# HKUDS/LLMRec

Measured on NVIDIA H100. Metric: train_interactions_per_sec, higher is better.
Workload: dtype f32

## Files before the change

llmrec_b200/csrc/dispatch.cu:

```cuda
#include <vector>
#include "common.cuh"

namespace llmrec {
int proj_fwd_simt(const float*, int64_t, const float*, const float*, float*, int64_t, int64_t, int, int, const int*, cudaStream_t);
int proj_fwd_simt(const uint16_t*, int64_t, const float*, const float*, float*, int64_t, int64_t, int, int, const int*, cudaStream_t);
int proj_wgrad_simt(const float*, int64_t, const float*, int64_t, float*, float*, int64_t, int, int, int, const int*, int64_t, cudaStream_t);
int proj_wgrad_simt(const uint16_t*, int64_t, const float*, int64_t, float*, float*, int64_t, int, int, int, const int*, int64_t, cudaStream_t);
int score_topk_simt(const float*, int64_t, const float*, int64_t, const int*, int, int, int, const int*, const int*, int, int*, float*, float*, int64_t, cudaStream_t);
bool proj_tc_supported(int d, int64_t ldx, const void* X, int k, bool wgrad, bool bf16);
int proj_fwd_tc_group(const llmrec_proj_fwd_problem*, const int32_t* const*, int, int, int, bool, cudaStream_t);
int proj_wgrad_tc_group(const llmrec_proj_wgrad_problem*, const int32_t* const*, const int64_t*, int, int, int, bool, float*, int64_t, cudaStream_t);
int64_t proj_wgrad_tc_scratch(const llmrec_proj_wgrad_problem*, int, int, bool);
bool score_tc_supported(int d, int K, long long ldu, long long ldi, const void* U, const void* I);
long long score_tc_scratch(int n_batch, int n_items, int d, int K);
int score_topk_tc(const float*, long long, const float*, long long, const int*, int, int, int, const int*, const int*, int, int*, float*, float*, long long, cudaStream_t);
}
using namespace llmrec;

static bool fwd_tc_ok(const llmrec_proj_fwd_problem* pr, int n, int d, int mode, bool bf16) {
  if (mode == 2 || n > 8) return false;
  for (int p = 0; p < n; ++p)
    if (!proj_tc_supported(d, pr[p].ldx, pr[p].X, pr[p].k, false, bf16) || pr[p].ldy % 4 != 0 || !aligned16(pr[p].Y) || !aligned16(pr[p].W) ||
        (pr[p].bias && !aligned16(pr[p].bias)) || ((mode == 0 || bf16) && !pr[p].wsplit))
      return false;
  return true;
}
static bool wg_tc_ok(const llmrec_proj_wgrad_problem* pr, int n, int d, int mode, bool bf16) {
  if (mode == 2 || n > 8) return false;
  for (int p = 0; p < n; ++p)
    if (!proj_tc_supported(d, pr[p].ldx, pr[p].X, pr[p].k, true, bf16) || pr[p].lddy % 4 != 0 || !aligned16(pr[p].dY)) return false;
  return true;
}

struct RowMaps { std::vector<const int32_t*> rows; std::vector<int64_t> n_dy; };
static int32_t flags(const llmrec_proj_fwd_problem& p) { return p._reserved; }
static int32_t flags(const llmrec_proj_fwd_problem_bf16& p) { return p._reserved; }
static int32_t flags(const llmrec_proj_wgrad_problem& p) { return p.accumulate; }
static int32_t flags(const llmrec_proj_wgrad_problem_bf16& p) { return p.accumulate; }
template <class Prob>
static int row_maps(const Prob* pr, int32_t n_prob, bool wgrad, RowMaps& M) {
  bool any = false;
  for (int p = 0; p < n_prob; ++p) any = any || (flags(pr[p]) & LLMREC_PROJ_ROW_MAP);
  if (!any) return 0;
  const llmrec_proj_row_map* rec = reinterpret_cast<const llmrec_proj_row_map*>(pr + n_prob);
  M.rows.assign(n_prob, nullptr);
  M.n_dy.assign(n_prob, 0);
  for (int p = 0; p < n_prob; ++p) {
    M.n_dy[p] = pr[p].n;
    if (!(flags(pr[p]) & LLMREC_PROJ_ROW_MAP)) continue;
    LLMREC_CHECK_ARG(rec[p].rows || pr[p].n <= 0, "proj: problem %d is flagged LLMREC_PROJ_ROW_MAP but its map is NULL", p);
    LLMREC_CHECK_ARG(!wgrad || rec[p].n_dy >= 0, "proj_wgrad: problem %d has a negative dY row count", p);
    M.rows[p] = rec[p].rows; M.n_dy[p] = rec[p].n_dy;
  }
  return 0;
}

static int proj_fwd_group(const llmrec_proj_fwd_problem* pr, const int32_t* const* rows, int32_t n_prob, int32_t d, int32_t mode, bool bf16,
                          llmrec_stream_t stream) {
  LLMREC_REQUIRE_DEVICE();
  LLMREC_CHECK_ARG(n_prob >= 1 && d >= 1, "proj_fwd_group: bad sizes");
  cudaStream_t st = as_stream(stream);
  for (int p0 = 0; p0 < n_prob; p0 += 8) {
    int np = n_prob - p0 < 8 ? n_prob - p0 : 8;
    if (fwd_tc_ok(pr + p0, np, d, mode, bf16)) {
      int rc = proj_fwd_tc_group(pr + p0, rows ? rows + p0 : nullptr, np, d, mode, bf16, st);
      if (rc) return rc;
    } else {
      for (int p = p0; p < p0 + np; ++p) {
        if (pr[p].n <= 0) continue;
        const int32_t* map = rows ? rows[p] : nullptr;
        int rc = bf16 ? proj_fwd_simt(reinterpret_cast<const uint16_t*>(pr[p].X), pr[p].ldx, pr[p].W, pr[p].bias, pr[p].Y, pr[p].ldy, pr[p].n, pr[p].k, d, map, st)
                      : proj_fwd_simt(pr[p].X, pr[p].ldx, pr[p].W, pr[p].bias, pr[p].Y, pr[p].ldy, pr[p].n, pr[p].k, d, map, st);
        if (rc) return rc;
      }
    }
  }
  return 0;
}
static std::vector<llmrec_proj_fwd_problem> as_f32_layout(const llmrec_proj_fwd_problem_bf16* pr, int32_t n_prob) {
  std::vector<llmrec_proj_fwd_problem> q(n_prob > 0 ? n_prob : 0);
  for (int p = 0; p < n_prob; ++p)
    q[p] = {reinterpret_cast<const float*>(pr[p].X), pr[p].W, pr[p].bias, pr[p].Y, pr[p].wsplit, pr[p].ldx, pr[p].ldy, pr[p].n, pr[p].k, 0};
  return q;
}
extern "C" int llmrec_proj_fwd_group_f32(const llmrec_proj_fwd_problem* pr, int32_t n_prob, int32_t d, int32_t mode, llmrec_stream_t stream) {
  LLMREC_CHECK_ARG(pr && n_prob >= 1, "proj_fwd_group: bad sizes");
  RowMaps M;
  if (int rc = row_maps(pr, n_prob, false, M)) return rc;
  return proj_fwd_group(pr, M.rows.empty() ? nullptr : M.rows.data(), n_prob, d, mode, false, stream);
}
extern "C" int llmrec_proj_fwd_group_bf16(const llmrec_proj_fwd_problem_bf16* pr, int32_t n_prob, int32_t d, int32_t mode, llmrec_stream_t stream) {
  LLMREC_CHECK_ARG(pr && n_prob >= 1, "proj_fwd_group: bad sizes");
  RowMaps M;
  if (int rc = row_maps(pr, n_prob, false, M)) return rc;
  return proj_fwd_group(as_f32_layout(pr, n_prob).data(), M.rows.empty() ? nullptr : M.rows.data(), n_prob, d, mode, true, stream);
}
extern "C" int llmrec_proj_fwd_f32(const float* X, int64_t ldx, const float* W, const float* bias, float* Y, int64_t ldy,
                                   int64_t n, int32_t k, int32_t d, int32_t mode, float* wsplit, llmrec_stream_t stream) {
  llmrec_proj_fwd_problem p{X, W, bias, Y, wsplit, ldx, ldy, n, k, 0};
  if (n <= 0) return 0;
  return llmrec_proj_fwd_group_f32(&p, 1, d, mode, stream);
}

static int64_t proj_wgrad_scratch(const llmrec_proj_wgrad_problem* pr, int32_t n_prob, int32_t d, int32_t mode, bool bf16) {
  int64_t need = 0;
  for (int p0 = 0; p0 < n_prob; p0 += 8) {
    int np = n_prob - p0 < 8 ? n_prob - p0 : 8;
    if (wg_tc_ok(pr + p0, np, d, mode, bf16)) { int64_t s = proj_wgrad_tc_scratch(pr + p0, np, d, bf16); need = s > need ? s : need; }
  }
  return need;
}
static int proj_wgrad_group(const llmrec_proj_wgrad_problem* pr, const int32_t* const* rows, const int64_t* n_dy, int32_t n_prob, int32_t d,
                            int32_t mode, bool bf16, float* scratch, int64_t scratch_elems, llmrec_stream_t stream) {
  LLMREC_REQUIRE_DEVICE();
  LLMREC_CHECK_ARG(n_prob >= 1 && d >= 1, "proj_wgrad_group: bad sizes");
  cudaStream_t st = as_stream(stream);
  for (int p0 = 0; p0 < n_prob; p0 += 8) {
    int np = n_prob - p0 < 8 ? n_prob - p0 : 8;
    if (wg_tc_ok(pr + p0, np, d, mode, bf16)) {
      int rc = proj_wgrad_tc_group(pr + p0, rows ? rows + p0 : nullptr, rows ? n_dy + p0 : nullptr, np, d, mode, bf16, scratch, scratch_elems, st);
      if (rc) return rc;
    } else {
      for (int p = p0; p < p0 + np; ++p) {
        const int acc = pr[p].accumulate & LLMREC_WGRAD_ACCUMULATE;
        const int32_t* map = rows ? rows[p] : nullptr;
        const int64_t ndy = n_dy ? n_dy[p] : pr[p].n;
        int rc = bf16 ? proj_wgrad_simt(reinterpret_cast<const uint16_t*>(pr[p].X), pr[p].ldx, pr[p].dY, pr[p].lddy, pr[p].dW, pr[p].db, pr[p].n, pr[p].k, d, acc, map, ndy, st)
                      : proj_wgrad_simt(pr[p].X, pr[p].ldx, pr[p].dY, pr[p].lddy, pr[p].dW, pr[p].db, pr[p].n, pr[p].k, d, acc, map, ndy, st);
        if (rc) return rc;
      }
    }
  }
  return 0;
}
static std::vector<llmrec_proj_wgrad_problem> as_f32_layout(const llmrec_proj_wgrad_problem_bf16* pr, int32_t n_prob) {
  std::vector<llmrec_proj_wgrad_problem> q(n_prob > 0 ? n_prob : 0);
  for (int p = 0; p < n_prob; ++p)
    q[p] = {reinterpret_cast<const float*>(pr[p].X), pr[p].dY, pr[p].dW, pr[p].db, pr[p].ldx, pr[p].lddy, pr[p].n, pr[p].k, pr[p].accumulate};
  return q;
}
extern "C" int64_t llmrec_proj_wgrad_group_scratch(const llmrec_proj_wgrad_problem* pr, int32_t n_prob, int32_t d, int32_t mode) {
  return proj_wgrad_scratch(pr, n_prob, d, mode, false);
}
extern "C" int64_t llmrec_proj_wgrad_group_bf16_scratch(const llmrec_proj_wgrad_problem_bf16* pr, int32_t n_prob, int32_t d, int32_t mode) {
  return proj_wgrad_scratch(as_f32_layout(pr, n_prob).data(), n_prob, d, mode, true);
}
extern "C" int llmrec_proj_wgrad_group_f32(const llmrec_proj_wgrad_problem* pr, int32_t n_prob, int32_t d, int32_t mode,
                                           float* scratch, int64_t scratch_elems, llmrec_stream_t stream) {
  LLMREC_CHECK_ARG(pr && n_prob >= 1, "proj_wgrad_group: bad sizes");
  RowMaps M;
  if (int rc = row_maps(pr, n_prob, true, M)) return rc;
  const bool mapped = !M.rows.empty();
  return proj_wgrad_group(pr, mapped ? M.rows.data() : nullptr, mapped ? M.n_dy.data() : nullptr, n_prob, d, mode, false, scratch, scratch_elems, stream);
}
extern "C" int llmrec_proj_wgrad_group_bf16(const llmrec_proj_wgrad_problem_bf16* pr, int32_t n_prob, int32_t d, int32_t mode,
                                            float* scratch, int64_t scratch_elems, llmrec_stream_t stream) {
  LLMREC_CHECK_ARG(pr && n_prob >= 1, "proj_wgrad_group: bad sizes");
  RowMaps M;
  if (int rc = row_maps(pr, n_prob, true, M)) return rc;
  const bool mapped = !M.rows.empty();
  return proj_wgrad_group(as_f32_layout(pr, n_prob).data(), mapped ? M.rows.data() : nullptr, mapped ? M.n_dy.data() : nullptr, n_prob, d, mode,
                          true, scratch, scratch_elems, stream);
}
extern "C" int64_t llmrec_proj_wgrad_scratch(int64_t n, int32_t k, int32_t d, int32_t mode) {
  llmrec_proj_wgrad_problem p{nullptr, nullptr, nullptr, nullptr, 4, 4, n, k, 0};
  if (mode == 2 || d % 32 != 0 || d > 256 || k % 4 != 0) return 0;
  return proj_wgrad_tc_scratch(&p, 1, d, false);
}
extern "C" int llmrec_proj_wgrad_f32(const float* X, int64_t ldx, const float* dY, int64_t lddy, float* dW, float* db,
                                     int64_t n, int32_t k, int32_t d, int32_t accumulate, int32_t mode,
                                     float* scratch, int64_t scratch_elems, llmrec_stream_t stream) {
  llmrec_proj_wgrad_problem p{X, dY, dW, db, ldx, lddy, n, k, accumulate};
  return llmrec_proj_wgrad_group_f32(&p, 1, d, mode, scratch, scratch_elems, stream);
}

extern "C" int64_t llmrec_score_topk_scratch(int32_t n_batch, int32_t n_items, int32_t d, int32_t K, int32_t mode) {
  if (mode != 2 && (d == 32 || d == 64 || d == 96 || d == 128) && K <= 64) return score_tc_scratch(n_batch, n_items, d, K);
  int64_t want = (int64_t)n_batch * n_items;
  int64_t cap = (int64_t)1 << 28;
  if (want > cap) want = (cap / n_items) * n_items;
  if (want < n_items) want = n_items;
  return want;
}
extern "C" int llmrec_score_topk_f32(const float* U, int64_t ldu, const float* I, int64_t ldi, const int32_t* users, int32_t n_batch,
                                     int32_t n_items, int32_t d, const int32_t* mask_rowptr, const int32_t* mask_col, int32_t K,
                                     int32_t* out_idx, float* out_val, int32_t mode, float* scratch, int64_t scratch_elems,
                                     llmrec_stream_t stream) {
  LLMREC_REQUIRE_DEVICE();
  LLMREC_CHECK_ARG(K >= 1 && K <= 64 && K <= n_items, "score_topk: K=%d unsupported (1..64, <= n_items)", K);
  if (n_batch <= 0) return 0;
  if (mode != 2 && score_tc_supported(d, K, ldu, ldi, U, I))
    return score_topk_tc(U, ldu, I, ldi, users, n_batch, n_items, d, mask_rowptr, mask_col, K, out_idx, out_val, scratch, scratch_elems, as_stream(stream));
  return score_topk_simt(U, ldu, I, ldi, users, n_batch, n_items, d, mask_rowptr, mask_col, K, out_idx, out_val, scratch, scratch_elems, as_stream(stream));
}
```

llmrec_b200/csrc/proj_tc.cu:

```cuda
#include <mutex>
#include <stdlib.h>
#include <vector>
#include <string.h>
#include "common.cuh"
#include "tc_common.cuh"
#include "proj_tc.cuh"

namespace llmrec {

using namespace tc;


typedef CUresult (*EncodeFn)(CUtensorMap*, CUtensorMapDataType, cuuint32_t, void*, const cuuint64_t*, const cuuint64_t*,
                             const cuuint32_t*, const cuuint32_t*, CUtensorMapInterleave, CUtensorMapSwizzle,
                             CUtensorMapL2promotion, CUtensorMapFloatOOBfill);

static EncodeFn get_encode() {
  static EncodeFn fn = nullptr;
  static bool tried = false;
  if (!tried) {
    tried = true;
    void* p = nullptr;
    cudaDriverEntryPointQueryResult q;
    if (cudaGetDriverEntryPoint("cuTensorMapEncodeTiled", &p, cudaEnableDefault, &q) == cudaSuccess && q == cudaDriverEntryPointSuccess)
      fn = reinterpret_cast<EncodeFn>(p);
  }
  return fn;
}

bool make_tmap_2d(CUtensorMap* out, CUtensorMapDataType dtype, const void* base, uint64_t inner, uint64_t outer, uint64_t row_stride_bytes,
                  uint32_t box_inner, uint32_t box_outer, bool swizzle128) {
  struct Entry { TmapKey k; CUtensorMap m; };
  static std::vector<Entry> cache;
  static std::mutex mu;
  TmapKey key{base, inner, outer, row_stride_bytes, box_inner, box_outer, swizzle128 ? 1u : 0u, (uint32_t)dtype};
  std::lock_guard<std::mutex> lock(mu);
  for (auto& e : cache)
    if (memcmp(&e.k, &key, sizeof(key)) == 0) { *out = e.m; return true; }
  EncodeFn enc = get_encode();
  if (!enc) { set_error("cuTensorMapEncodeTiled entry point unavailable"); return false; }
  cuuint64_t dims[2] = {inner, outer};
  cuuint64_t strides[1] = {row_stride_bytes};
  cuuint32_t box[2] = {box_inner, box_outer};
  cuuint32_t estr[2] = {1, 1};
  CUresult r = enc(out, dtype, 2, const_cast<void*>(base), dims, strides, box, estr,
                   CU_TENSOR_MAP_INTERLEAVE_NONE, swizzle128 ? CU_TENSOR_MAP_SWIZZLE_128B : CU_TENSOR_MAP_SWIZZLE_NONE, CU_TENSOR_MAP_L2_PROMOTION_L2_256B,
                   CU_TENSOR_MAP_FLOAT_OOB_FILL_NONE);
  if (r != CUDA_SUCCESS) { set_error("cuTensorMapEncodeTiled failed (%d) inner=%llu outer=%llu stride=%llu box=%ux%u", (int)r,
                                     (unsigned long long)inner, (unsigned long long)outer, (unsigned long long)row_stride_bytes, box_inner, box_outer); return false; }
  if (cache.size() > 256) cache.clear();
  cache.push_back({key, *out});
  return true;
}

__device__ __forceinline__ uint8_t* align1024(uint8_t* p) {
  return reinterpret_cast<uint8_t*>((reinterpret_cast<uintptr_t>(p) + 1023) & ~uintptr_t(1023));
}

constexpr uint32_t kSmemMax = 227u * 1024u;
constexpr int kProducerRegs = 40, kConsumerRegs = 232;

template <int D, bool SPLIT, int MB, bool BF16 = false>
struct ProjCfg {
  static constexpr int TM = tile_m(MB);
  static constexpr int NB = SPLIT ? (BF16 ? 3 : 2) : 1;
  static constexpr uint32_t kX = TM * 128u;
  static constexpr uint32_t kB = D * 128u;
  static constexpr uint32_t kStage = kX + kB * NB;
  static constexpr int kFit = (int)((kSmemMax - 1024u - 256u) / kStage);
  static constexpr int kStages = kFit > 4 ? 4 : kFit;
  static constexpr uint32_t kSmem = 1024u  + kStages * kStage + 2u * kStages * 8u;
  static_assert(kStages >= 2, "projection ring needs two stages");
};

__device__ __forceinline__ void ld_frag_fwd(uint32_t (&a)[4], uint32_t sx, int blk, int kk, int warp, int lane) {
  const int g = lane >> 2, t = lane & 3;
  const uint32_t row = sx + (blk * 64 + warp * 16 + g) * 128 + t * 4;
  const uint32_t c0 = ((2 * kk) ^ g) << 4, c1 = c0 ^ 16;
  a[0] = lds_u32(row + c0);
  a[1] = lds_u32(row + 1024 + c0);
  a[2] = lds_u32(row + c1);
  a[3] = lds_u32(row + 1024 + c1);
}
__device__ __forceinline__ int wgrad_feature(int blk, int warp, int h, int g) {
  return blk * 64 + 32 * (warp >> 1) + 8 * (warp & 1) + 4 * h + (g & 3) + 16 * (g >> 2);
}
__device__ __forceinline__ void ld_frag_wgrad(uint32_t (&a)[4], uint32_t sx, int blk, int kk, int warp, int lane) {
  const int g = lane >> 2, t = lane & 3;
  const uint32_t base = sx + (blk * 2 + (warp >> 1)) * 4096 + kk * 1024 + t * 128 + (g & 3) * 4;
  const uint32_t q = (2 * (warp & 1) + 4 * (g >> 2)) ^ t;
  a[0] = lds_u32(base + (q << 4));
  a[1] = lds_u32(base + ((q ^ 1) << 4));
  a[2] = lds_u32(base + 512 + ((q ^ 4) << 4));
  a[3] = lds_u32(base + 512 + ((q ^ 5) << 4));
}

template <int D, bool SPLIT, int MB, bool BF16 = false>
struct FwdUnit {
  using Cfg = ProjCfg<D, SPLIT, MB, BF16>;
  static constexpr int kTransA = 0;
  const FwdParams& P; int p, mblk, kb_n;
  __device__ FwdUnit(const FwdParams& P_, int u) : P(P_) {
    p = 0;
    while (p + 1 < P.n_prob && u >= P.prob[p + 1].tile_start) ++p;
    mblk = u - P.prob[p].tile_start;
    kb_n = P.prob[p].kblocks;
  }
  __device__ void issue(uint8_t* st, uint64_t* bar, int kb, uint64_t pol) const {
    constexpr int bk = stage_k(BF16);
    tma_load_2d_hint(st, &P.tmA[p], bar, kb * bk, mblk * Cfg::TM, pol);
#pragma unroll
    for (int i = 0; i < Cfg::NB; ++i) tma_load_2d(st + Cfg::kX + i * Cfg::kB, &P.tmW[p], bar, kb * bk, i * D);
  }
  static __device__ void ld_frag(uint32_t (&a)[4], uint32_t sx, int blk, int kk, int warp, int lane) { ld_frag_fwd(a, sx, blk, kk, warp, lane); }
  static __device__ uint64_t a_desc(uint32_t sx, int blk, int kk) { return gmma_desc_sw128(sx + blk * 8192u + kk * 32u); }
  __device__ void store(float (&acc)[MB][D / 2], int cw, int warp, int lane) const {
    const FwdProblem& pr = P.prob[p];
    const int g = lane >> 2, t = lane & 3;
#pragma unroll
    for (int j = 0; j < MB; ++j) {
      const int row0 = mblk * Cfg::TM + (cw * MB + j) * 64 + warp * 16 + g;
      long long yrow[2];
#pragma unroll
      for (int h = 0; h < 2; ++h) {
        const int row = row0 + 8 * h;
        yrow[h] = row < pr.n ? (pr.rows ? (long long)__ldg(pr.rows + row) : (long long)row) : -1;
      }
#pragma unroll
      for (int c = 0; c < D / 8; ++c) {
        const int col = c * 8 + 2 * t;
        const float2 b = pr.bias ? __ldg(reinterpret_cast<const float2*>(pr.bias + col)) : make_float2(0.f, 0.f);
#pragma unroll
        for (int h = 0; h < 2; ++h) {
          if (yrow[h] >= 0)
            *reinterpret_cast<float2*>(pr.Y + yrow[h] * pr.ldy + col) = make_float2(acc[j][4 * c + 2 * h] + b.x, acc[j][4 * c + 2 * h + 1] + b.y);
        }
      }
    }
  }
};

template <int D, bool SPLIT, int MB, bool BF16 = false>
struct WgUnit {
  using Cfg = ProjCfg<D, SPLIT, MB, BF16>;
  static constexpr int kBk = stage_k(BF16);
  static constexpr int kTransA = 1;
  const WgParams& P; int p, u, ft, r0, kb_n;
  __device__ WgUnit(const WgParams& P_, int u_) : P(P_), u(u_) {
    p = 0;
    while (p + 1 < P.n_prob && u >= P.prob[p + 1].item_start) ++p;
    const WgProblem& pr = P.prob[p];
    const int local = u - pr.item_start, chunk = local / pr.ft_tiles;
    ft = local - chunk * pr.ft_tiles;
    r0 = chunk * pr.rows_per_chunk;
    kb_n = (min(pr.n, r0 + pr.rows_per_chunk) - r0 + kBk - 1) / kBk;
  }
  __device__ void issue(uint8_t* st, uint64_t* bar, int kb, uint64_t pol) const {
    const int r = r0 + kb * kBk;
    if constexpr (BF16) {
#pragma unroll
      for (int b = 0; b < Cfg::TM / 64; ++b) tma_load_2d_hint(st + b * 8192, &P.tmX[p], bar, ft * Cfg::TM + 64 * b, r, pol);
    } else {
#pragma unroll
      for (int b = 0; b < Cfg::TM / 32; ++b) tma_load_2d_hint(st + b * 4096, &P.tmX[p], bar, ft * Cfg::TM + 32 * b, r, pol);
    }
#pragma unroll
    for (int i = 0; i < Cfg::NB; ++i) tma_load_2d(st + Cfg::kX + i * Cfg::kB, &P.tmG[p], bar, r, i * D);
  }
  static __device__ void ld_frag(uint32_t (&a)[4], uint32_t sx, int blk, int kk, int warp, int lane) { ld_frag_wgrad(a, sx, blk, kk, warp, lane); }
  static __device__ uint64_t a_desc(uint32_t sx, int blk, int kk) { return gmma_desc_sw128_mn(sx + blk * 8192u + kk * 2048u); }
  __device__ void store(float (&acc)[MB][D / 2], int cw, int warp, int lane) const {
    const int g = lane >> 2, t = lane & 3;
    float* out = P.partial + (long long)u * Cfg::TM * D;
#pragma unroll
    for (int j = 0; j < MB; ++j)
#pragma unroll
      for (int h = 0; h < 2; ++h) {
        const int f = BF16 ? (cw * MB + j) * 64 + warp * 16 + 8 * h + g : wgrad_feature(cw * MB + j, warp, h, g);
        float* o = out + (long long)f * D + 2 * t;
#pragma unroll
        for (int c = 0; c < D / 8; ++c) *reinterpret_cast<float2*>(o + c * 8) = make_float2(acc[j][4 * c + 2 * h], acc[j][4 * c + 2 * h + 1]);
      }
  }
};

template <int D, bool SPLIT, int MB, bool BF16, class Unit, class Params>
__device__ __forceinline__ void proj_pipeline(const Params& P, int total) {
  using Cfg = ProjCfg<D, SPLIT, MB, BF16>;
  extern __shared__ uint8_t smem_raw[];
  uint8_t* smem = align1024(smem_raw);
  uint64_t* full = reinterpret_cast<uint64_t*>(smem + Cfg::kStages * Cfg::kStage);
  uint64_t* empty = full + Cfg::kStages;
  const int tid = threadIdx.x, wg = tid >> 7, warp = (tid >> 5) & 3, lane = tid & 31;
  if (tid == 0) {
    for (int s = 0; s < Cfg::kStages; ++s) { mbar_init(&full[s], 1); mbar_init(&empty[s], 8); }
    fence_barrier_init();
  }
  __syncthreads();

  if (wg == 0) {
    setmaxnreg_dec<kProducerRegs>();
    if (tid == 0) {
      const uint64_t pol = l2_policy_evict_first();
      int s = 0; uint32_t ph = 0;
      for (int u = blockIdx.x; u < total; u += gridDim.x) {
        const Unit w(P, u);
        for (int kb = 0; kb < w.kb_n; ++kb) {
          mbar_wait(&empty[s], ph ^ 1u);
          mbar_arrive_expect_tx(&full[s], Cfg::kStage);
          w.issue(smem + s * Cfg::kStage, &full[s], kb, pol);
          if (++s == Cfg::kStages) { s = 0; ph ^= 1u; }
        }
      }
    }
    return;
  }

  setmaxnreg_inc<kConsumerRegs>();
  const int cw = wg - 1;
  int s = 0; uint32_t ph = 0;
  float acc[MB][D / 2];
  for (int u = blockIdx.x; u < total; u += gridDim.x) {
    const Unit w(P, u);
#pragma unroll
    for (int j = 0; j < MB; ++j)
#pragma unroll
      for (int i = 0; i < D / 2; ++i) acc[j][i] = 0.f;
    int prev = -1;
    for (int kb = 0; kb < w.kb_n; ++kb) {
      mbar_wait(&full[s], ph);
      const uint32_t st = smem_u32(smem + s * Cfg::kStage), bh = st + Cfg::kX, bl = bh + Cfg::kB;
      if constexpr (BF16) {
#pragma unroll
        for (int kk = 0; kk < 4; ++kk) {
          wgmma_fence();
#pragma unroll
          for (int j = 0; j < MB; ++j) {
            const uint64_t a = Unit::a_desc(st, cw * MB + j, kk);
            if (SPLIT) {
              WgmmaSSbf16<D, Unit::kTransA>::mma(acc[j], a, gmma_desc_sw128(bl + Cfg::kB + kk * 32u));
              WgmmaSSbf16<D, Unit::kTransA>::mma(acc[j], a, gmma_desc_sw128(bl + kk * 32u));
            }
            WgmmaSSbf16<D, Unit::kTransA>::mma(acc[j], a, gmma_desc_sw128(bh + kk * 32u));
          }
          wgmma_commit();
          wgmma_wait<1>();
          if (kk == 0 && prev >= 0 && lane == 0) mbar_arrive(&empty[prev]);
        }
      } else {
#pragma unroll
        for (int kk = 0; kk < 4; ++kk) {
          uint32_t ah[MB][4], al[MB][4];
#pragma unroll
          for (int j = 0; j < MB; ++j) {
            Unit::ld_frag(ah[j], st, cw * MB + j, kk, warp, lane);
            if (SPLIT)
#pragma unroll
              for (int i = 0; i < 4; ++i) {
                const float x = __uint_as_float(ah[j][i]), hi = tf32_hi(x);
                ah[j][i] = __float_as_uint(hi);
                al[j][i] = __float_as_uint(x - hi);
              }
          }
          wgmma_fence();
          const uint64_t dh = gmma_desc_sw128(bh + kk * 32u);
#pragma unroll
          for (int j = 0; j < MB; ++j) {
            if (SPLIT) {
              WgmmaRS<D>::mma(acc[j], al[j], dh);
              WgmmaRS<D>::mma(acc[j], ah[j], gmma_desc_sw128(bl + kk * 32u));
            }
            WgmmaRS<D>::mma(acc[j], ah[j], dh);
          }
          wgmma_commit();
          wgmma_wait<1>();
          if (kk == 0 && prev >= 0 && lane == 0) mbar_arrive(&empty[prev]);
        }
      }
      prev = s;
      if (++s == Cfg::kStages) { s = 0; ph ^= 1u; }
    }
    wgmma_wait<0>();
    if (prev >= 0 && lane == 0) mbar_arrive(&empty[prev]);
    w.store(acc, cw, warp, lane);
  }
}

template <int D, bool SPLIT, int MB, bool BF16>
__global__ void __launch_bounds__(384, 1) proj_fwd_tc_kernel(const __grid_constant__ FwdParams P) {
  proj_pipeline<D, SPLIT, MB, BF16, FwdUnit<D, SPLIT, MB, BF16>>(P, P.total_tiles);
}

template <int D, bool SPLIT, int MB, bool BF16>
__global__ void __launch_bounds__(384, 1) proj_wgrad_tc_kernel(const __grid_constant__ WgParams P) {
  proj_pipeline<D, SPLIT, MB, BF16, WgUnit<D, SPLIT, MB, BF16>>(P, P.total_items);
}

static int num_sms() {
  static int n[64] = {};
  int dev = 0;
  if (cudaGetDevice(&dev) != cudaSuccess || dev < 0 || dev >= 64) return 132;
  if (!n[dev] && cudaDeviceGetAttribute(&n[dev], cudaDevAttrMultiProcessorCount, dev) != cudaSuccess) n[dev] = 132;
  return n[dev];
}

static int pick_mb(int d, long long units_at_256) { return d <= 128 && units_at_256 >= num_sms() ? 2 : 1; }

template <int D, bool SPLIT, int MB, bool BF16>
static int launch_fwd(const FwdParams& P, cudaStream_t st) {
  using Cfg = ProjCfg<D, SPLIT, MB, BF16>;
  LLMREC_CHECK_CUDA(cudaFuncSetAttribute(proj_fwd_tc_kernel<D, SPLIT, MB, BF16>, cudaFuncAttributeMaxDynamicSharedMemorySize, (int)Cfg::kSmem));
  const int grid = P.total_tiles < num_sms() ? P.total_tiles : num_sms();
  proj_fwd_tc_kernel<D, SPLIT, MB, BF16><<<grid, 384, Cfg::kSmem, st>>>(P);
  LLMREC_CHECK_LAUNCH("proj_fwd_tc");
  return 0;
}

template <int D, bool SPLIT, int MB, bool BF16>
static int launch_wgrad(const WgParams& P, cudaStream_t st) {
  using Cfg = ProjCfg<D, SPLIT, MB, BF16>;
  LLMREC_CHECK_CUDA(cudaFuncSetAttribute(proj_wgrad_tc_kernel<D, SPLIT, MB, BF16>, cudaFuncAttributeMaxDynamicSharedMemorySize, (int)Cfg::kSmem));
  const int grid = P.total_items < num_sms() ? P.total_items : num_sms();
  proj_wgrad_tc_kernel<D, SPLIT, MB, BF16><<<grid, 384, Cfg::kSmem, st>>>(P);
  LLMREC_CHECK_LAUNCH("proj_wgrad_tc");
  return 0;
}

template <int D, bool SPLIT, bool BF16>
static int launch_fwd_mb(const FwdParams& P, int mb, cudaStream_t st) {
  if constexpr (D <= 128) { if (mb == 2) return launch_fwd<D, SPLIT, 2, BF16>(P, st); }
  return launch_fwd<D, SPLIT, 1, BF16>(P, st);
}
template <int D, bool SPLIT, bool BF16>
static int launch_wgrad_mb(const WgParams& P, int mb, cudaStream_t st) {
  if constexpr (D <= 128) { if (mb == 2) return launch_wgrad<D, SPLIT, 2, BF16>(P, st); }
  return launch_wgrad<D, SPLIT, 1, BF16>(P, st);
}

#define LLMREC_PROJ_WIDTHS(X) X(32) X(64) X(96) X(128) X(160) X(192) X(224) X(256)

static int fwd_launch(const FwdParams& P, bool split, int mb, bool bf16, cudaStream_t st) {
  switch (P.d) {
#define LLMREC_CASE(W) case W: \
    if (bf16) return split ? launch_fwd_mb<W, true, true>(P, mb, st) : launch_fwd_mb<W, false, true>(P, mb, st); \
    return split ? launch_fwd_mb<W, true, false>(P, mb, st) : launch_fwd_mb<W, false, false>(P, mb, st);
    LLMREC_PROJ_WIDTHS(LLMREC_CASE)
#undef LLMREC_CASE
  }
  set_error("proj_fwd: no tensor-core kernel for d=%d", P.d);
  return 1;
}

static int wgrad_launch(const WgParams& P, bool split, int mb, bool bf16, cudaStream_t st) {
  switch (P.d) {
#define LLMREC_CASE(W) case W: \
    if (bf16) return split ? launch_wgrad_mb<W, true, true>(P, mb, st) : launch_wgrad_mb<W, false, true>(P, mb, st); \
    return split ? launch_wgrad_mb<W, true, false>(P, mb, st) : launch_wgrad_mb<W, false, false>(P, mb, st);
    LLMREC_PROJ_WIDTHS(LLMREC_CASE)
#undef LLMREC_CASE
  }
  set_error("proj_wgrad: no tensor-core kernel for d=%d", P.d);
  return 1;
}

struct DytParams { const float* dY[kMaxProb]; long long ld[kMaxProb]; int n[kMaxProb]; float* out[kMaxProb]; long long ldt[kMaxProb];
                   const int* rows[kMaxProb]; int d, split; };
template <bool BF16>
__global__ void __launch_bounds__(256) dyt_split_kernel(const DytParams P) {
  __shared__ float tile[32][33];
  const int p = blockIdx.z, n = P.n[p], r0 = blockIdx.x * 32, e0 = blockIdx.y * 32;
  if (r0 >= n) return;
  const int tx = threadIdx.x & 31, ty = threadIdx.x >> 5;
  const float* __restrict__ src = P.dY[p];
  const int* __restrict__ rows = P.rows[p];
#pragma unroll
  for (int i = ty; i < 32; i += 8) {
    const int r = r0 + i;
    tile[i][tx] = r < n ? __ldg(src + (long long)(rows ? __ldg(rows + r) : r) * P.ld[p] + e0 + tx) : 0.f;
  }
  __syncthreads();
  if (r0 + tx >= n) return;
  const long long ldt = P.ldt[p], lo = (long long)P.d * ldt;
#pragma unroll
  for (int i = ty; i < 32; i += 8) {
    const float v = tile[tx][i];
    const long long at = (long long)(e0 + i) * ldt + r0 + tx;
    if constexpr (BF16) {
      uint16_t* o = reinterpret_cast<uint16_t*>(P.out[p]) + at;
      if (P.split) bf16_split3(v, o[0], o[lo], o[2 * lo]);
      else o[0] = bf16_bits(bf16_trunc(v));
    } else {
      float* o = P.out[p] + at;
      if (P.split) { const float h = tf32_hi(v); o[0] = h; o[lo] = v - h; }
      else o[0] = v;
    }
  }
}

struct WsplitParams { const float* W[kMaxProb]; float* out[kMaxProb]; long long n[kMaxProb]; };
__global__ void wsplit_kernel(const WsplitParams P) {
  const float* __restrict__ W = P.W[blockIdx.y];
  float* __restrict__ out = P.out[blockIdx.y];
  const long long n = P.n[blockIdx.y];
  for (long long i = blockIdx.x * (long long)blockDim.x + threadIdx.x; i < n; i += (long long)gridDim.x * blockDim.x) {
    const float v = W[i]; const float h = tf32_hi(v); out[i] = h; out[n + i] = v - h;
  }
}
__global__ void wsplit_bf16_kernel(const WsplitParams P, int split) {
  const float* __restrict__ W = P.W[blockIdx.y];
  uint16_t* __restrict__ out = reinterpret_cast<uint16_t*>(P.out[blockIdx.y]);
  const long long n = P.n[blockIdx.y];
  for (long long i = blockIdx.x * (long long)blockDim.x + threadIdx.x; i < n; i += (long long)gridDim.x * blockDim.x) {
    if (split) bf16_split3(W[i], out[i], out[n + i], out[2 * n + i]);
    else out[i] = bf16_bits(bf16_trunc(W[i]));
  }
}

struct ReduceOut { float* dW; int k, n_src, accumulate, blk_start; int src[kMaxProb]; };
struct ReduceParams { ReduceOut out[kMaxProb]; int n_out; int d, tm; const float* partial; WgProblem prob[kMaxProb]; };
__global__ void __launch_bounds__(256) wgrad_reduce_kernel(const ReduceParams R) {
  __shared__ float4 part[4][64];
  int o = 0;
  while (o + 1 < R.n_out && (int)blockIdx.x >= R.out[o + 1].blk_start) ++o;
  const ReduceOut ro = R.out[o];
  const int d = R.d, f4_per_feat = d >> 2;
  const int feats_per_blk = 64 / f4_per_feat;
  const int local = blockIdx.x - ro.blk_start;
  const int tm = R.tm, groups_per_ft = tm / feats_per_blk;
  const int ft = local / groups_per_ft, fg = local - ft * groups_per_ft;
  const int e = threadIdx.x & 63, sl = threadIdx.x >> 6;
  const bool owned = e < feats_per_blk * f4_per_feat;
  const int f = fg * feats_per_blk + e / f4_per_feat;
  const int dc4 = e - (e / f4_per_feat) * f4_per_feat;
  float4 s = make_float4(0.f, 0.f, 0.f, 0.f);
  int idx = 0;
  for (int j = 0; owned && j < ro.n_src; ++j) {
    const WgProblem pr = R.prob[ro.src[j]];
#pragma unroll 4
    for (int c = 0; c < pr.chunks; ++c, ++idx) {
      if ((idx & 3) != sl) continue;
      const float4 v = __ldg(reinterpret_cast<const float4*>(R.partial + ((long long)(pr.item_start + c * pr.ft_tiles + ft) * tm + f) * d) + dc4);
      s.x += v.x; s.y += v.y; s.z += v.z; s.w += v.w;
    }
  }
  part[sl][e] = s;
  __syncthreads();
  if (sl == 0 && owned) {
    float4 a = part[0][e], b = part[1][e], c = part[2][e], g = part[3][e];
    float4 t = make_float4((a.x + b.x) + (c.x + g.x), (a.y + b.y) + (c.y + g.y), (a.z + b.z) + (c.z + g.z), (a.w + b.w) + (c.w + g.w));
    const int gf = ft * tm + f;
    if (gf < ro.k) {
      float* p = ro.dW + (long long)(dc4 * 4) * ro.k + gf;
      if (ro.accumulate) { t.x += p[0]; t.y += p[ro.k]; t.z += p[2LL * ro.k]; t.w += p[3LL * ro.k]; }
      p[0] = t.x; p[ro.k] = t.y; p[2LL * ro.k] = t.z; p[3LL * ro.k] = t.w;
    }
  }
}

struct ColsumParams { const float* dY[kMaxProb]; long long ld[kMaxProb]; long long n[kMaxProb]; float* db[kMaxProb]; int acc[kMaxProb]; int d; int n_prob; float* partial; unsigned* ticket; };
constexpr int kColsumSlices = 128;
__global__ void __launch_bounds__(256) colsum_kernel(const ColsumParams P) {
  __shared__ float red[256];
  __shared__ bool s_last;
  const int p = blockIdx.y, b = blockIdx.x, d = P.d;
  const int groups = 256 / d > 0 ? 256 / d : 1;
  const int g = threadIdx.x / d, c = threadIdx.x - g * d;
  float s = 0.f;
  if (g < groups && P.db[p]) {
#pragma unroll 4
    for (long long r = (long long)b * groups + g; r < P.n[p]; r += (long long)kColsumSlices * groups) s += __ldg(P.dY[p] + r * P.ld[p] + c);
  }
  red[threadIdx.x] = (g < groups) ? s : 0.f;
  __syncthreads();
  if (threadIdx.x < d) {
    float t = 0.f;
    for (int gg = 0; gg < groups; ++gg) t += red[gg * d + threadIdx.x];
    P.partial[((long long)p * kColsumSlices + b) * d + threadIdx.x] = t;
  }
  __threadfence();
  __syncthreads();
  if (threadIdx.x == 0) s_last = atomicAdd(P.ticket, 1u) == gridDim.x * gridDim.y - 1;
  __syncthreads();
  if (!s_last) return;
  __threadfence();
  for (int q = 0; q < P.n_prob; ++q) {
    if (!P.db[q]) continue;
    float t = 0.f;
    if (g < groups)
      for (int bb = g; bb < kColsumSlices; bb += groups) t += __ldcg(P.partial + ((long long)q * kColsumSlices + bb) * d + c);
    __syncthreads();
    red[threadIdx.x] = (g < groups) ? t : 0.f;
    __syncthreads();
    if (threadIdx.x < d) {
      float u = 0.f;
      for (int gg = 0; gg < groups; ++gg) u += red[gg * d + threadIdx.x];
      float* o = P.db[q] + threadIdx.x;
      *o = P.acc[q] ? (*o + u) : u;
    }
  }
  if (threadIdx.x == 0) *P.ticket = 0u;
}

bool proj_tc_supported(int d, int64_t ldx, const void* X, int k, bool wgrad, bool bf16) {
  (void)wgrad;
  const int q = bf16 ? 8 : 4;
  return d % 32 == 0 && d >= 32 && d <= 256 && ldx % q == 0 && aligned16(X) && k >= 1 && k % q == 0;
}

static CUtensorMapDataType x_type(bool bf16) { return bf16 ? CU_TENSOR_MAP_DATA_TYPE_BFLOAT16 : CU_TENSOR_MAP_DATA_TYPE_FLOAT32; }

int proj_fwd_tc_group(const llmrec_proj_fwd_problem* pr, const int32_t* const* rows, int n_prob, int d, int mode, bool bf16, cudaStream_t st) {
  const bool split = (mode == 0);
  const bool need_ws = split || bf16;
  const int es = bf16 ? 2 : 4, bk = stage_k(bf16);
  FwdParams P;
  memset(&P, 0, sizeof(P));
  P.n_prob = n_prob; P.d = d;
  WsplitParams WS;
  memset(&WS, 0, sizeof(WS));
  int n_ws = 0;
  long long ws_max = 0, tiles256 = 0;
  for (int p = 0; p < n_prob; ++p) tiles256 += (pr[p].n + tile_m(2) - 1) / tile_m(2);
  const int mb = pick_mb(d, tiles256), tm = tile_m(mb);
  int tiles = 0;
  for (int p = 0; p < n_prob; ++p) {
    const float* wsrc = need_ws ? pr[p].wsplit : pr[p].W;
    LLMREC_CHECK_ARG(!need_ws || pr[p].wsplit, "proj_fwd: 3xTF32 mode and bf16 X need a wsplit buffer of 2*d*k floats");
    bool fresh = true;
    for (int q = 0; q < p; ++q) fresh = fresh && !(pr[q].W == pr[p].W && pr[q].wsplit == pr[p].wsplit);
    if (need_ws && fresh) {
      WS.W[n_ws] = pr[p].W; WS.out[n_ws] = pr[p].wsplit; WS.n[n_ws] = (long long)d * pr[p].k;
      ws_max = WS.n[n_ws] > ws_max ? WS.n[n_ws] : ws_max;
      ++n_ws;
    }
    if (pr[p].n > 0) {
      const int pieces = split ? (bf16 ? 3 : 2) : 1;
      if (!make_tmap_2d(&P.tmA[p], x_type(bf16), pr[p].X, (uint64_t)pr[p].k, (uint64_t)pr[p].n, (uint64_t)pr[p].ldx * es, bk, (uint32_t)tm)) return 4;
      if (!make_tmap_2d(&P.tmW[p], x_type(bf16), wsrc, (uint64_t)pr[p].k, (uint64_t)(pieces * d), (uint64_t)pr[p].k * es, bk, (uint32_t)d)) return 4;
    }
    P.prob[p].n = (int)pr[p].n; P.prob[p].k = pr[p].k; P.prob[p].kblocks = (pr[p].k + bk - 1) / bk;
    P.prob[p].tile_start = tiles; P.prob[p].ldy = pr[p].ldy; P.prob[p].Y = pr[p].Y; P.prob[p].bias = pr[p].bias;
    P.prob[p].rows = rows ? rows[p] : nullptr;
    tiles += (int)((pr[p].n + tm - 1) / tm);
  }
  P.total_tiles = tiles;
  if (n_ws > 0) {
    if (bf16) wsplit_bf16_kernel<<<dim3((unsigned)((ws_max + 255) / 256), n_ws), 256, 0, st>>>(WS, split ? 1 : 0);
    else wsplit_kernel<<<dim3((unsigned)((ws_max + 255) / 256), n_ws), 256, 0, st>>>(WS);
    LLMREC_CHECK_LAUNCH("wsplit");
  }
  if (tiles <= 0) return 0;
  return fwd_launch(P, split, mb, bf16, st);
}

static int wg_rows_per_chunk(int64_t n) {
  int r = 2048;
  while (r > 256 && n / r < 4) r >>= 1;
  return r;
}

struct WgPlan { WgProblem prob[kMaxProb]; int items, mb, tm; int64_t ldt[kMaxProb], dyt[kMaxProb], colsum, total; };
static void wg_plan(const llmrec_proj_wgrad_problem* pr, int n_prob, int d, bool bf16, WgPlan& W) {
  long long items256 = 0;
  for (int p = 0; p < n_prob; ++p) {
    const int rpc = wg_rows_per_chunk(pr[p].n);
    items256 += (long long)((pr[p].k + tile_m(2) - 1) / tile_m(2)) * ((pr[p].n + rpc - 1) / rpc);
  }
  W.mb = pick_mb(d, items256); W.tm = tile_m(W.mb);
  W.items = 0;
  for (int p = 0; p < n_prob; ++p) {
    WgProblem& w = W.prob[p];
    w.n = (int)pr[p].n; w.k = pr[p].k; w.ft_tiles = (pr[p].k + W.tm - 1) / W.tm;
    w.rows_per_chunk = wg_rows_per_chunk(pr[p].n);
    w.chunks = (int)((pr[p].n + w.rows_per_chunk - 1) / w.rows_per_chunk);
    w.item_start = W.items;
    W.items += w.ft_tiles * w.chunks;
  }
  W.colsum = 4 + (int64_t)W.items * W.tm * d;
  int64_t off = W.colsum + (int64_t)n_prob * kColsumSlices * d;
  for (int p = 0; p < n_prob; ++p) {
    W.ldt[p] = bf16 ? (pr[p].n + 7) & ~int64_t(7) : (pr[p].n + 3) & ~int64_t(3);
    W.dyt[p] = off;
    off += 2 * (int64_t)d * W.ldt[p];
  }
  W.total = off;
}

int64_t proj_wgrad_tc_scratch(const llmrec_proj_wgrad_problem* pr, int n_prob, int d, bool bf16) {
  WgPlan W;
  wg_plan(pr, n_prob, d, bf16, W);
  return W.total;
}

int proj_wgrad_tc_group(const llmrec_proj_wgrad_problem* pr, const int32_t* const* rows, const int64_t* n_dy, int n_prob, int d, int mode,
                        bool bf16, float* scratch, int64_t scratch_elems, cudaStream_t st) {
  const bool split = (mode == 0);
  const int es = bf16 ? 2 : 4, bk = stage_k(bf16), pieces = split ? (bf16 ? 3 : 2) : 1;
  WgPlan W;
  wg_plan(pr, n_prob, d, bf16, W);
  LLMREC_CHECK_ARG(scratch && scratch_elems >= W.total, "proj_wgrad: scratch too small (%lld < %lld)", (long long)scratch_elems, (long long)W.total);
  WgParams P;
  memset(&P, 0, sizeof(P));
  P.n_prob = n_prob; P.d = d; P.total_items = W.items;
  P.partial = scratch + 4;
  ColsumParams C;
  memset(&C, 0, sizeof(C));
  C.d = d; C.n_prob = n_prob; C.partial = scratch + W.colsum;
  C.ticket = reinterpret_cast<unsigned*>(scratch);
  DytParams T;
  memset(&T, 0, sizeof(T));
  T.d = d; T.split = split ? 1 : 0;
  int64_t n_max = 0;
  for (int p = 0; p < n_prob; ++p) {
    P.prob[p] = W.prob[p];
    float* dyt = scratch + W.dyt[p];
    if (pr[p].n > 0) {
      if (!make_tmap_2d(&P.tmX[p], x_type(bf16), pr[p].X, (uint64_t)pr[p].k, (uint64_t)pr[p].n, (uint64_t)pr[p].ldx * es, bk, bk)) return 4;
      if (!make_tmap_2d(&P.tmG[p], x_type(bf16), dyt, (uint64_t)pr[p].n, (uint64_t)(pieces * d), (uint64_t)W.ldt[p] * es, bk, (uint32_t)d)) return 4;
    }
    const int32_t* map = rows ? rows[p] : nullptr;
    T.dY[p] = pr[p].dY; T.ld[p] = pr[p].lddy; T.n[p] = (int)pr[p].n; T.out[p] = dyt; T.ldt[p] = W.ldt[p]; T.rows[p] = map;
    n_max = pr[p].n > n_max ? pr[p].n : n_max;
    C.dY[p] = pr[p].dY; C.ld[p] = pr[p].lddy; C.n[p] = n_dy ? n_dy[p] : pr[p].n; C.db[p] = pr[p].db;
    C.acc[p] = pr[p].accumulate & LLMREC_WGRAD_ACCUMULATE;
  }
  bool any_db = false;
  for (int p = 0; p < n_prob; ++p) any_db = any_db || pr[p].db != nullptr;
  static const bool branches = !(getenv("LLMREC_BRANCHES") && atoi(getenv("LLMREC_BRANCHES")) == 0);
  struct Branch { cudaStream_t side; cudaEvent_t fork, join; };
  static Branch per_device[64] = {};
  int dev = 0;
  LLMREC_CHECK_CUDA(cudaGetDevice(&dev));
  LLMREC_CHECK_ARG(dev >= 0 && dev < 64, "proj_wgrad: device ordinal %d out of range", dev);
  cudaStream_t& side = per_device[dev].side;
  cudaEvent_t& ev_fork = per_device[dev].fork;
  cudaEvent_t& ev_join = per_device[dev].join;
  bool forked = false;
  if (any_db) {
    cudaStream_t cs = st;
    if (branches) {
      if (!side) {
        LLMREC_CHECK_CUDA(cudaStreamCreateWithFlags(&side, cudaStreamNonBlocking));
        LLMREC_CHECK_CUDA(cudaEventCreateWithFlags(&ev_fork, cudaEventDisableTiming));
        LLMREC_CHECK_CUDA(cudaEventCreateWithFlags(&ev_join, cudaEventDisableTiming));
      }
      LLMREC_CHECK_CUDA(cudaEventRecord(ev_fork, st));
      LLMREC_CHECK_CUDA(cudaStreamWaitEvent(side, ev_fork, 0));
      cs = side; forked = true;
    }
    colsum_kernel<<<dim3(kColsumSlices, n_prob), 256, 0, cs>>>(C);
    LLMREC_CHECK_LAUNCH("colsum");
    if (forked) LLMREC_CHECK_CUDA(cudaEventRecord(ev_join, side));
  }
  if (W.items > 0) {
    const dim3 grid((unsigned)((n_max + 31) / 32), (unsigned)(d / 32), (unsigned)n_prob);
    if (bf16) dyt_split_kernel<true><<<grid, 256, 0, st>>>(T);
    else dyt_split_kernel<false><<<grid, 256, 0, st>>>(T);
    LLMREC_CHECK_LAUNCH("dyt_split");
    int rc = wgrad_launch(P, split, W.mb, bf16, st);
    if (rc) return rc;
  }
  ReduceParams R;
  memset(&R, 0, sizeof(R));
  R.d = d; R.tm = W.tm; R.partial = scratch + 4;
  int blocks = 0;
  for (int p = 0; p < n_prob; ++p) {
    R.prob[p] = P.prob[p];
    int o = -1;
    for (int q = 0; q < R.n_out; ++q) if (R.out[q].dW == pr[p].dW) o = q;
    if (o < 0) {
      o = R.n_out++;
      R.out[o].dW = pr[p].dW; R.out[o].k = pr[p].k; R.out[o].accumulate = pr[p].accumulate & LLMREC_WGRAD_ACCUMULATE; R.out[o].n_src = 0;
    }
    LLMREC_CHECK_ARG(R.out[o].k == pr[p].k, "proj_wgrad: problems sharing dW must share k");
    R.out[o].src[R.out[o].n_src++] = p;
  }
  const int feats_per_blk = 64 / (d / 4);
  for (int o = 0; o < R.n_out; ++o) { R.out[o].blk_start = blocks; blocks += ((R.out[o].k + W.tm - 1) / W.tm) * (W.tm / feats_per_blk); }
  wgrad_reduce_kernel<<<blocks, 256, 0, st>>>(R);
  LLMREC_CHECK_LAUNCH("wgrad_reduce");
  if (forked) LLMREC_CHECK_CUDA(cudaStreamWaitEvent(st, ev_join, 0));
  return 0;
}

}
```

llmrec_b200/csrc/proj_tc.cuh:

```cuda
#pragma once
#include "tc_common.cuh"

namespace llmrec {

constexpr int kMaxProb = 8;
constexpr int BK = 32;
constexpr int BK16 = 64;
constexpr int stage_k(bool bf16) { return bf16 ? BK16 : BK; }
constexpr int tile_m(int mb) { return 128 * mb; }

struct FwdProblem { int n, k, kblocks, tile_start; long long ldy; float* Y; const float* bias; const int* rows; };
struct FwdParams {
  CUtensorMap tmA[kMaxProb];
  CUtensorMap tmW[kMaxProb];
  FwdProblem prob[kMaxProb];
  int n_prob, total_tiles, d;
};

struct WgProblem { int n, k, ft_tiles, chunks, rows_per_chunk, item_start; };
struct WgParams {
  CUtensorMap tmX[kMaxProb];
  CUtensorMap tmG[kMaxProb];
  WgProblem prob[kMaxProb];
  int n_prob, total_items, d;
  float* partial;
};

}
```

Before: 1.296 million.

## Build split dY operand in-kernel with producer builder warps instead of transpose pass

Result: faster. 1.337 million, median of 6 (+3.1%).

```diff
diff --git a/llmrec_b200/csrc/dispatch.cu b/llmrec_b200/csrc/dispatch.cu
--- a/llmrec_b200/csrc/dispatch.cu
+++ b/llmrec_b200/csrc/dispatch.cu
@@ -10,7 +10,7 @@
 bool proj_tc_supported(int d, int64_t ldx, const void* X, int k, bool wgrad, bool bf16);
 int proj_fwd_tc_group(const llmrec_proj_fwd_problem*, const int32_t* const*, int, int, int, bool, cudaStream_t);
 int proj_wgrad_tc_group(const llmrec_proj_wgrad_problem*, const int32_t* const*, const int64_t*, int, int, int, bool, float*, int64_t, cudaStream_t);
-int64_t proj_wgrad_tc_scratch(const llmrec_proj_wgrad_problem*, int, int, bool);
+int64_t proj_wgrad_tc_scratch(const llmrec_proj_wgrad_problem*, int, int, int, bool);
 bool score_tc_supported(int d, int K, long long ldu, long long ldi, const void* U, const void* I);
 long long score_tc_scratch(int n_batch, int n_items, int d, int K);
 int score_topk_tc(const float*, long long, const float*, long long, const int*, int, int, int, const int*, const int*, int, int*, float*, float*, long long, cudaStream_t);
@@ -106,7 +106,7 @@
   int64_t need = 0;
   for (int p0 = 0; p0 < n_prob; p0 += 8) {
     int np = n_prob - p0 < 8 ? n_prob - p0 : 8;
-    if (wg_tc_ok(pr + p0, np, d, mode, bf16)) { int64_t s = proj_wgrad_tc_scratch(pr + p0, np, d, bf16); need = s > need ? s : need; }
+    if (wg_tc_ok(pr + p0, np, d, mode, bf16)) { int64_t s = proj_wgrad_tc_scratch(pr + p0, np, d, mode, bf16); need = s > need ? s : need; }
   }
   return need;
 }
@@ -165,7 +165,7 @@
 extern "C" int64_t llmrec_proj_wgrad_scratch(int64_t n, int32_t k, int32_t d, int32_t mode) {
   llmrec_proj_wgrad_problem p{nullptr, nullptr, nullptr, nullptr, 4, 4, n, k, 0};
   if (mode == 2 || d % 32 != 0 || d > 256 || k % 4 != 0) return 0;
-  return proj_wgrad_tc_scratch(&p, 1, d, false);
+  return proj_wgrad_tc_scratch(&p, 1, d, mode, false);
 }
 extern "C" int llmrec_proj_wgrad_f32(const float* X, int64_t ldx, const float* dY, int64_t lddy, float* dW, float* db,
                                      int64_t n, int32_t k, int32_t d, int32_t accumulate, int32_t mode,
diff --git a/llmrec_b200/csrc/proj_tc.cu b/llmrec_b200/csrc/proj_tc.cu
--- a/llmrec_b200/csrc/proj_tc.cu
+++ b/llmrec_b200/csrc/proj_tc.cu
@@ -58,7 +58,6 @@
 }
 
 constexpr uint32_t kSmemMax = 227u * 1024u;
-constexpr int kProducerRegs = 40, kConsumerRegs = 232;
 
 template <int D, bool SPLIT, int MB, bool BF16 = false>
 struct ProjCfg {
@@ -99,6 +98,9 @@
 struct FwdUnit {
   using Cfg = ProjCfg<D, SPLIT, MB, BF16>;
   static constexpr int kTransA = 0;
+  static constexpr int kBuilders = 0;
+  static constexpr int kProducerRegs = 40, kConsumerRegs = 232;
+  static constexpr uint32_t kTx = Cfg::kStage;
   const FwdParams& P; int p, mblk, kb_n;
   __device__ FwdUnit(const FwdParams& P_, int u) : P(P_) {
     p = 0;
@@ -155,6 +157,10 @@
     r0 = chunk * pr.rows_per_chunk;
     kb_n = (min(pr.n, r0 + pr.rows_per_chunk) - r0 + kBk - 1) / kBk;
   }
+  static constexpr int kBuilders = SPLIT && !BF16 ? 3 : 0;
+  static constexpr int kProducerRegs = kBuilders ? 72 : 40;
+  static constexpr int kConsumerRegs = kBuilders ? 216 : 232;
+  static constexpr uint32_t kTx = kBuilders ? Cfg::kX : Cfg::kStage;
   __device__ void issue(uint8_t* st, uint64_t* bar, int kb, uint64_t pol) const {
     const int r = r0 + kb * kBk;
     if constexpr (BF16) {
@@ -164,8 +170,42 @@
 #pragma unroll
       for (int b = 0; b < Cfg::TM / 32; ++b) tma_load_2d_hint(st + b * 4096, &P.tmX[p], bar, ft * Cfg::TM + 32 * b, r, pol);
     }
-#pragma unroll
-    for (int i = 0; i < Cfg::NB; ++i) tma_load_2d(st + Cfg::kX + i * Cfg::kB, &P.tmG[p], bar, r, i * D);
+    if constexpr (kBuilders == 0) {
+#pragma unroll
+      for (int i = 0; i < Cfg::NB; ++i) tma_load_2d(st + Cfg::kX + i * Cfg::kB, &P.tmG[p], bar, r, i * D);
+    }
+  }
+  static constexpr int kTasks = D / 8;
+  static constexpr int kBatch = 3;
+  __device__ void build(uint8_t* st, int kb, int bw, int lane) const {
+    const int n = P.prob[p].n, r = r0 + kb * kBk + lane;
+    const int* __restrict__ map = P.rows[p];
+    const float* src = r < n ? P.dY[p] + (long long)(map ? __ldg(map + r) : r) * P.lddy[p] : nullptr;
+    uint8_t* b = st + Cfg::kX + (lane & 3) * 4;
+    const int q = lane >> 2;
+    for (int t0 = bw; t0 < kTasks; t0 += kBuilders * kBatch) {
+      float4 v[kBatch][2];
+#pragma unroll
+      for (int j = 0; j < kBatch; ++j) {
+        const int t = t0 + kBuilders * j;
+#pragma unroll
+        for (int h = 0; h < 2; ++h)
+          v[j][h] = t < kTasks && src ? __ldg(reinterpret_cast<const float4*>(src + 8 * t + 4 * h)) : make_float4(0.f, 0.f, 0.f, 0.f);
+      }
+#pragma unroll
+      for (int j = 0; j < kBatch; ++j) {
+        const int t = t0 + kBuilders * j;
+        if (t >= kTasks) break;
+#pragma unroll
+        for (int e = 0; e < 8; ++e) {
+          const float4 w = v[j][e >> 2];
+          const float x = (e & 3) == 0 ? w.x : (e & 3) == 1 ? w.y : (e & 3) == 2 ? w.z : w.w, hi = tf32_hi(x);
+          uint8_t* o = b + (8 * t + e) * 128 + ((q ^ e) & 7) * 16;
+          *reinterpret_cast<float*>(o) = hi;
+          *reinterpret_cast<float*>(o + Cfg::kB) = x - hi;
+        }
+      }
+    }
   }
   static __device__ void ld_frag(uint32_t (&a)[4], uint32_t sx, int blk, int kk, int warp, int lane) { ld_frag_wgrad(a, sx, blk, kk, warp, lane); }
   static __device__ uint64_t a_desc(uint32_t sx, int blk, int kk) { return gmma_desc_sw128_mn(sx + blk * 8192u + kk * 2048u); }
@@ -193,13 +233,14 @@
   uint64_t* empty = full + Cfg::kStages;
   const int tid = threadIdx.x, wg = tid >> 7, warp = (tid >> 5) & 3, lane = tid & 31;
   if (tid == 0) {
-    for (int s = 0; s < Cfg::kStages; ++s) { mbar_init(&full[s], 1); mbar_init(&empty[s], 8); }
+    for (int s = 0; s < Cfg::kStages; ++s) { mbar_init(&full[s], 1 + Unit::kBuilders); mbar_init(&empty[s], 8); }
     fence_barrier_init();
   }
   __syncthreads();
 
+  static_assert(128 * Unit::kProducerRegs + 256 * Unit::kConsumerRegs <= 384 * 168, "setmaxnreg split exceeds the CTA's registers");
   if (wg == 0) {
-    setmaxnreg_dec<kProducerRegs>();
+    setmaxnreg_dec<Unit::kProducerRegs>();
     if (tid == 0) {
       const uint64_t pol = l2_policy_evict_first();
       int s = 0; uint32_t ph = 0;
@@ -207,16 +248,32 @@
         const Unit w(P, u);
         for (int kb = 0; kb < w.kb_n; ++kb) {
           mbar_wait(&empty[s], ph ^ 1u);
-          mbar_arrive_expect_tx(&full[s], Cfg::kStage);
+          mbar_arrive_expect_tx(&full[s], Unit::kTx);
           w.issue(smem + s * Cfg::kStage, &full[s], kb, pol);
           if (++s == Cfg::kStages) { s = 0; ph ^= 1u; }
         }
       }
     }
+    if constexpr (Unit::kBuilders > 0) {
+      if (warp >= 1) {
+        int s = 0; uint32_t ph = 0;
+        for (int u = blockIdx.x; u < total; u += gridDim.x) {
+          const Unit w(P, u);
+          for (int kb = 0; kb < w.kb_n; ++kb) {
+            mbar_wait(&empty[s], ph ^ 1u);
+            w.build(smem + s * Cfg::kStage, kb, warp - 1, lane);
+            fence_proxy_async_smem();
+            __syncwarp();
+            if (lane == 0) mbar_arrive(&full[s]);
+            if (++s == Cfg::kStages) { s = 0; ph ^= 1u; }
+          }
+        }
+      }
+    }
     return;
   }
 
-  setmaxnreg_inc<kConsumerRegs>();
+  setmaxnreg_inc<Unit::kConsumerRegs>();
   const int cw = wg - 1;
   int s = 0; uint32_t ph = 0;
   float acc[MB][D / 2];
@@ -380,19 +437,18 @@
   }
   __syncthreads();
   if (r0 + tx >= n) return;
-  const long long ldt = P.ldt[p], lo = (long long)P.d * ldt;
+  const long long ldt = P.ldt[p];
 #pragma unroll
   for (int i = ty; i < 32; i += 8) {
     const float v = tile[tx][i];
     const long long at = (long long)(e0 + i) * ldt + r0 + tx;
     if constexpr (BF16) {
       uint16_t* o = reinterpret_cast<uint16_t*>(P.out[p]) + at;
+      const long long lo = (long long)P.d * ldt;
       if (P.split) bf16_split3(v, o[0], o[lo], o[2 * lo]);
       else o[0] = bf16_bits(bf16_trunc(v));
     } else {
-      float* o = P.out[p] + at;
-      if (P.split) { const float h = tf32_hi(v); o[0] = h; o[lo] = v - h; }
-      else o[0] = v;
+      P.out[p][at] = v;
     }
   }
 }
@@ -560,7 +616,8 @@
 }
 
 struct WgPlan { WgProblem prob[kMaxProb]; int items, mb, tm; int64_t ldt[kMaxProb], dyt[kMaxProb], colsum, total; };
-static void wg_plan(const llmrec_proj_wgrad_problem* pr, int n_prob, int d, bool bf16, WgPlan& W) {
+static bool wg_builds_b(int mode, bool bf16) { return mode == 0 && !bf16; }
+static void wg_plan(const llmrec_proj_wgrad_problem* pr, int n_prob, int d, int mode, bool bf16, WgPlan& W) {
   long long items256 = 0;
   for (int p = 0; p < n_prob; ++p) {
     const int rpc = wg_rows_per_chunk(pr[p].n);
@@ -581,14 +638,14 @@
   for (int p = 0; p < n_prob; ++p) {
     W.ldt[p] = bf16 ? (pr[p].n + 7) & ~int64_t(7) : (pr[p].n + 3) & ~int64_t(3);
     W.dyt[p] = off;
-    off += 2 * (int64_t)d * W.ldt[p];
+    if (!wg_builds_b(mode, bf16)) off += 2 * (int64_t)d * W.ldt[p];
   }
   W.total = off;
 }
 
-int64_t proj_wgrad_tc_scratch(const llmrec_proj_wgrad_problem* pr, int n_prob, int d, bool bf16) {
+int64_t proj_wgrad_tc_scratch(const llmrec_proj_wgrad_problem* pr, int n_prob, int d, int mode, bool bf16) {
   WgPlan W;
-  wg_plan(pr, n_prob, d, bf16, W);
+  wg_plan(pr, n_prob, d, mode, bf16, W);
   return W.total;
 }
 
@@ -596,8 +653,9 @@
                         bool bf16, float* scratch, int64_t scratch_elems, cudaStream_t st) {
   const bool split = (mode == 0);
   const int es = bf16 ? 2 : 4, bk = stage_k(bf16), pieces = split ? (bf16 ? 3 : 2) : 1;
+  const bool build_b = wg_builds_b(mode, bf16);
   WgPlan W;
-  wg_plan(pr, n_prob, d, bf16, W);
+  wg_plan(pr, n_prob, d, mode, bf16, W);
   LLMREC_CHECK_ARG(scratch && scratch_elems >= W.total, "proj_wgrad: scratch too small (%lld < %lld)", (long long)scratch_elems, (long long)W.total);
   WgParams P;
   memset(&P, 0, sizeof(P));
@@ -613,12 +671,14 @@
   int64_t n_max = 0;
   for (int p = 0; p < n_prob; ++p) {
     P.prob[p] = W.prob[p];
+    const int32_t* map = rows ? rows[p] : nullptr;
     float* dyt = scratch + W.dyt[p];
     if (pr[p].n > 0) {
       if (!make_tmap_2d(&P.tmX[p], x_type(bf16), pr[p].X, (uint64_t)pr[p].k, (uint64_t)pr[p].n, (uint64_t)pr[p].ldx * es, bk, bk)) return 4;
-      if (!make_tmap_2d(&P.tmG[p], x_type(bf16), dyt, (uint64_t)pr[p].n, (uint64_t)(pieces * d), (uint64_t)W.ldt[p] * es, bk, (uint32_t)d)) return 4;
-    }
-    const int32_t* map = rows ? rows[p] : nullptr;
+      if (!build_b &&
+          !make_tmap_2d(&P.tmG[p], x_type(bf16), dyt, (uint64_t)pr[p].n, (uint64_t)(pieces * d), (uint64_t)W.ldt[p] * es, bk, (uint32_t)d)) return 4;
+    }
+    P.dY[p] = pr[p].dY; P.lddy[p] = pr[p].lddy; P.rows[p] = map;
     T.dY[p] = pr[p].dY; T.ld[p] = pr[p].lddy; T.n[p] = (int)pr[p].n; T.out[p] = dyt; T.ldt[p] = W.ldt[p]; T.rows[p] = map;
     n_max = pr[p].n > n_max ? pr[p].n : n_max;
     C.dY[p] = pr[p].dY; C.ld[p] = pr[p].lddy; C.n[p] = n_dy ? n_dy[p] : pr[p].n; C.db[p] = pr[p].db;
@@ -653,10 +713,12 @@
     if (forked) LLMREC_CHECK_CUDA(cudaEventRecord(ev_join, side));
   }
   if (W.items > 0) {
-    const dim3 grid((unsigned)((n_max + 31) / 32), (unsigned)(d / 32), (unsigned)n_prob);
-    if (bf16) dyt_split_kernel<true><<<grid, 256, 0, st>>>(T);
-    else dyt_split_kernel<false><<<grid, 256, 0, st>>>(T);
-    LLMREC_CHECK_LAUNCH("dyt_split");
+    if (!build_b) {
+      const dim3 grid((unsigned)((n_max + 31) / 32), (unsigned)(d / 32), (unsigned)n_prob);
+      if (bf16) dyt_split_kernel<true><<<grid, 256, 0, st>>>(T);
+      else dyt_split_kernel<false><<<grid, 256, 0, st>>>(T);
+      LLMREC_CHECK_LAUNCH("dyt_split");
+    }
     int rc = wgrad_launch(P, split, W.mb, bf16, st);
     if (rc) return rc;
   }
diff --git a/llmrec_b200/csrc/proj_tc.cuh b/llmrec_b200/csrc/proj_tc.cuh
--- a/llmrec_b200/csrc/proj_tc.cuh
+++ b/llmrec_b200/csrc/proj_tc.cuh
@@ -21,6 +21,9 @@
 struct WgParams {
   CUtensorMap tmX[kMaxProb];
   CUtensorMap tmG[kMaxProb];
+  const float* dY[kMaxProb];
+  long long lddy[kMaxProb];
+  const int* rows[kMaxProb];
   WgProblem prob[kMaxProb];
   int n_prob, total_items, d;
   float* partial;
```
